# neuroailab/CounterfactualWorldModels

Measured on AMD Instinct MI355X. Metric: predicted frames/sec (2x224x224, ViT-B/8), higher is better.
Workload: dtype bf16; 1 GPU; ViT-base VMAE 8x8, batch=32 synthetic frame pairs (BASELINE configs[1]); predictor=base_8x8patch_2frames_1tube, per_gpu_batch=32, global_batch=32, n_vis=792, mode=parity, lanes=2 (the batch runs as two half batches on two HIP streams inside the library), arithmetic=split-bf16 (hi+lo) MFMA operands, 3 MFMAs/product, fp32 accumulate, parallelism=dp1 (independent frame pairs per rank, no collective), weights=random-init (deterministic synthetic generator)

## Files before the change

counterfactualworldmodels_amd/csrc/attention.hip:

```cpp
#include "attention_tail.h"

namespace cwm {

template <int PLANES>
__global__ __launch_bounds__(256, 2) void attention_kernel(const AttnParams p) {
    constexpr int TILE_BYTES = 64 * 64 * 2;
    constexpr int STAGE_BYTES = TILE_BYTES * 2 * PLANES;
    extern __shared__ __attribute__((aligned(16))) char smem[];

    const int tid = threadIdx.x;
    const int lane = tid & 63;
    const int wave = __builtin_amdgcn_readfirstlane(tid >> 6);
    const int qcol = lane & 31, hh = lane >> 5;
    const int N = p.n_tok;
    int qt, bh;
    attn_tile_of_block(p.n_q > 0 ? p.n_q : p.n_tok, 128, p.remap != 0, qt, bh);
    if (attention_is_split_tail(p, qt, gridDim.x, p.n_q > 0 ? p.n_q : p.n_tok)) {
        attention_tail_block<PLANES>(p, smem, bh, qt * 128, p.n_q > 0 ? p.n_q : p.n_tok);
        return;
    }
    const int b = bh / p.heads, h = bh - b * p.heads;
    const int q0 = qt * 128 + wave * 32;
    const int NQ = p.n_q > 0 ? p.n_q : p.n_tok;
    const bool active = q0 < NQ;
// ... 45 lines not shown
#pragma unroll
                for (int pl = 0; pl < PLANES; ++pl) kfr[kb][s][pl] = *reinterpret_cast<const bf16x8*>(base + pl * TILE_BYTES + k_off[kb][s]);
        __builtin_amdgcn_sched_barrier(0);
        f32x16 sacc[2];
#pragma unroll
        for (int kb = 0; kb < 2; ++kb) {
#pragma unroll
            for (int r = 0; r < 16; ++r) sacc[kb][r] = 0.f;
#pragma unroll
            for (int s = 0; s < 4; ++s) mfma_split<PLANES>(sacc[kb], kfr[kb][s][0], kfr[kb][s][PLANES - 1], qf[0][s], qf[PLANES - 1][s]);
        }
        __builtin_amdgcn_sched_barrier(0);
        bf16x4 vfr[4][2][PLANES][2];
#pragma unroll
        for (int ks = 0; ks < 4; ++ks)
#pragma unroll
            for (int db = 0; db < 2; ++db)
#pragma unroll
                for (int pl = 0; pl < PLANES; ++pl) {
                    const char* vb = base + (PLANES + pl) * TILE_BYTES + v_base[db] + ks * 2048;
                    vfr[ks][db][pl][0] = lds_read_tr16(vb);
                    vfr[ks][db][pl][1] = lds_read_tr16(vb + 1024);
                }
        __builtin_amdgcn_sched_barrier(0);

        if constexpr (LAST) {
            if (N & 63) {
#pragma unroll
                for (int kb = 0; kb < 2; ++kb) mask_rows_from(sacc[kb], kt * 64 + kb * 32, hh, N);
            }
        }
        float mx = sacc[0][0];
#pragma unroll
        for (int kb = 0; kb < 2; ++kb)
#pragma unroll
            for (int r = 0; r < 16; ++r) mx = fmaxf(mx, sacc[kb][r]);
        mx = max_lane_xor32(mx);
        const float m_new = fmaxf(m_run, mx);
        const bool grew = __any(m_new > m_run);
        const float alpha = grew ? __builtin_amdgcn_exp2f((m_run - m_new) * kLog2e) : 1.0f;
        m_run = m_new;
        const float mc = m_new * kLog2e;
        float rowsum = 0.f;
#pragma unroll
        for (int kb = 0; kb < 2; ++kb)
#pragma unroll
            for (int r = 0; r < 16; ++r) {
                const float pv = __builtin_amdgcn_exp2f(fmaf(sacc[kb][r], kLog2e, -mc));
                sacc[kb][r] = pv;
                rowsum += pv;
            }
        l_run = l_run * alpha + rowsum;
        if (grew) {
#pragma unroll
            for (int db = 0; db < 2; ++db)
#pragma unroll
                for (int r = 0; r < 16; ++r) oacc[db][r] *= alpha;
        }

#pragma unroll
        for (int ks = 0; ks < 4; ++ks) {
            const int kb = ks >> 1, s = ks & 1;
            bf16x8 ph, plo;
            p_fragments<PLANES>(sacc[kb], s, ph, plo);
#pragma unroll
            for (int db = 0; db < 2; ++db) mfma_split<PLANES>(oacc[db], join_halves(vfr[ks][db][0]), join_halves(vfr[ks][db][PLANES - 1]), ph, plo);
        }
        }

        if constexpr (!LAST) {
            store_tiles(cur ^ 1);
            __syncthreads();
        }
    };
    for (int kt = 0; kt + 1 < nkt; ++kt) tile_step(kt, std::false_type{});
    tile_step(nkt - 1, std::true_type{});

    const float l_tot = l_run + __shfl_xor(l_run, 32, 64);
    const float inv = 1.0f / l_tot;
    const int q = q0 + qcol;
    if (q < NQ) {
        const int64_t orow = (int64_t)b * NQ + q;
#pragma unroll
        for (int db = 0; db < 2; ++db) store_o_block<PLANES>(p.o, orow, p.ldo, h * 64 + db * 32, oacc[db], inv, hh);
    }
}

int launch_attention(const AttnParams& p_in, int planes, hipStream_t stream) {
    AttnParams p = p_in;
    const Tuning& tn = p.tune ? *p.tune : default_tuning();
    p.remap = tn.attn_remap;
    p.tail_split = tn.attn_tail;
    CWM_REQUIRE(planes == 1 || planes == 2, "attention: planes must be 1 or 2");
    CWM_REQUIRE(p.n_tok > 0 && p.batch > 0 && p.heads > 0, "attention: empty problem");
    CWM_REQUIRE(p.ldo % 4 == 0, "attention: ldo must be a multiple of 4");
    CWM_REQUIRE((int64_t)p.n_tok * 128 < (1ll << 31), "attention: %d tokens exceed the 32-bit tile offsets within one (batch, head)", p.n_tok);
    CWM_REQUIRE(p.q_off >= 0 && p.n_q >= 0 && p.q_off + p.n_q <= p.n_tok, "attention: query rows [%d, %d) outside the %d tokens", p.q_off, p.q_off + p.n_q, p.n_tok);
    const int nqb = ((p.n_q > 0 ? p.n_q : p.n_tok) + 127) / 128;
    const int kern = tn.attn_kernel ? tn.attn_kernel : (p.n_tok >= (planes == 2 ? 160 : 512) ? 3 : 1);
    if (kern == 3) return launch_attention_pipe(p, planes, stream);
    CWM_REQUIRE(kern == 1, "attention: unknown kernel %d (1: 4-wave, 3: software-pipelined)", kern);
    const dim3 grid(nqb, p.batch * p.heads);
    const size_t smem = (size_t)2 * (64 * 64 * 2) * 2 * planes;
    if (planes == 1) {
        hipLaunchKernelGGL(attention_kernel<1>, grid, dim3(256), smem, stream, p);
    } else {
        if (int rc = cwm_set_max_lds((const void*)attention_kernel<2>, (int)smem)) return rc;
        hipLaunchKernelGGL(attention_kernel<2>, grid, dim3(256), smem, stream, p);
    }
    CWM_HIP_CHECK(hipGetLastError());
    return 0;
}

}
```

counterfactualworldmodels_amd/csrc/attention_device.h:

```cpp
#pragma once
#include "common.h"
#include "kernels.h"
#include <type_traits>

namespace cwm {

__device__ __forceinline__ void attn_tile_of_item(int L, int nqb, int nbh, int nq, int rows, bool remap, int& qt, int& bh) {
    qt = L % nqb;
    bh = L / nqb;
    if (nbh % 8 != 0 || !remap) return;
    const int xcd = L & 7, idx = L >> 3, per = nbh >> 3;
    const int light = (nqb > 1 && (nq - (nqb - 1) * rows) * 2 <= rows) ? 1 : 0;
    const int heavy = nqb - light;
    if (idx < per * heavy) {
        bh = xcd * per + idx / heavy;
        qt = idx - (idx / heavy) * heavy;
    } else {
        bh = xcd * per + (idx - per * heavy);
        qt = nqb - 1;
    }
}
__device__ __forceinline__ void attn_tile_of_block(int nq, int rows, bool remap, int& qt, int& bh) {
    attn_tile_of_item(blockIdx.y * gridDim.x + blockIdx.x, gridDim.x, gridDim.y, nq, rows, remap, qt, bh);
}

__device__ __forceinline__ int lds_off128(int row, int chunk) { return row * 128 + ((chunk ^ ((row >> 1) & 7)) << 4); }
__device__ __forceinline__ int lds_off_v(int row, int chunk) { return row * 128 + ((chunk ^ (((row >> 1) & 1) << 2)) << 4); }

typedef __attribute__((ext_vector_type(4))) short s16x4;
__device__ __forceinline__ bf16x4 lds_read_tr16(const char* ptr) {
    typedef __attribute__((address_space(3))) s16x4 lds_s16x4;
    const s16x4 v = __builtin_amdgcn_ds_read_tr16_b64_v4i16((lds_s16x4*)ptr);
    return __builtin_bit_cast(bf16x4, v);
}
__device__ __forceinline__ bf16x8 join_halves(const bf16x4 (&h)[2]) { return __builtin_shufflevector(h[0], h[1], 0, 1, 2, 3, 4, 5, 6, 7); }

typedef __attribute__((ext_vector_type(2))) unsigned int u32x2;
template <int OFF>
__device__ __forceinline__ u32x2 lds_read_tr16_asm(unsigned addr) {
    u32x2 v;
    asm volatile("ds_read_b64_tr_b16 %0, %1 offset:%2" : "=v"(v) : "v"(addr), "n"(OFF) : "memory");
    return v;
}
template <int KS, int PLANES>
__device__ __forceinline__ void lds_read_v_step(u32x2 (&dst)[2][PLANES][2], unsigned va0, unsigned va1) {
    constexpr int T = 64 * 64 * 2;
    dst[0][0][0] = lds_read_tr16_asm<KS * 2048>(va0);
    dst[0][0][1] = lds_read_tr16_asm<KS * 2048 + 1024>(va0);
    if constexpr (PLANES == 2) {
        dst[0][PLANES - 1][0] = lds_read_tr16_asm<KS * 2048 + T>(va0);
        dst[0][PLANES - 1][1] = lds_read_tr16_asm<KS * 2048 + T + 1024>(va0);
    }
    dst[1][0][0] = lds_read_tr16_asm<KS * 2048>(va1);
    dst[1][0][1] = lds_read_tr16_asm<KS * 2048 + 1024>(va1);
    if constexpr (PLANES == 2) {
        dst[1][PLANES - 1][0] = lds_read_tr16_asm<KS * 2048 + T>(va1);
        dst[1][PLANES - 1][1] = lds_read_tr16_asm<KS * 2048 + T + 1024>(va1);
    }
}

template <int N, int PLANES>
__device__ __forceinline__ void lds_wait_v_step(u32x2 (&v)[2][PLANES][2]) {
    if constexpr (PLANES == 2)
        asm volatile("s_waitcnt lgkmcnt(%8)"
                     : "+v"(v[0][0][0]), "+v"(v[0][0][1]), "+v"(v[0][1][0]), "+v"(v[0][1][1]), "+v"(v[1][0][0]), "+v"(v[1][0][1]), "+v"(v[1][1][0]), "+v"(v[1][1][1])
                     : "n"(N)
                     : "memory");
    else
        asm volatile("s_waitcnt lgkmcnt(%4)" : "+v"(v[0][0][0]), "+v"(v[0][0][1]), "+v"(v[1][0][0]), "+v"(v[1][0][1]) : "n"(N) : "memory");
}

__device__ __forceinline__ float max_lane_xor32(float x) {
    const auto sw = __builtin_amdgcn_permlane32_swap(__float_as_uint(x), __float_as_uint(x), false, false);
    return fmaxf(__uint_as_float(sw[0]), __uint_as_float(sw[1]));
}

__device__ __forceinline__ float sum_lane_xor32(float x) {
    const auto sw = __builtin_amdgcn_permlane32_swap(__float_as_uint(x), __float_as_uint(x), false, false);
    return __uint_as_float(sw[0]) + __uint_as_float(sw[1]);
}


template <int PLANES>
__device__ __forceinline__ void mfma_split(f32x16& acc, const bf16x8& a_hi, const bf16x8& a_lo, const bf16x8& b_hi, const bf16x8& b_lo) {
    if constexpr (PLANES == 2) {
        acc = __builtin_amdgcn_mfma_f32_32x32x16_bf16(a_lo, b_hi, acc, 0, 0, 0);
        acc = __builtin_amdgcn_mfma_f32_32x32x16_bf16(a_hi, b_lo, acc, 0, 0, 0);
    }
    acc = __builtin_amdgcn_mfma_f32_32x32x16_bf16(a_hi, b_hi, acc, 0, 0, 0);
}

template <int PLANES>
__device__ __forceinline__ void p_fragments(const f32x16& s, int ks, bf16x8& ph, bf16x8& plo) {
#pragma unroll
    for (int j = 0; j < 8; ++j) split_bf16_at<PLANES>(s[8 * ks + j], ph, plo, j);
}

__device__ __forceinline__ int acc_row(int r, int hh) { return (r & 3) + 8 * (r >> 2) + 4 * hh; }
__device__ __forceinline__ void mask_rows_from(f32x16& s, int row0, int hh, int limit) {
#pragma unroll
    for (int r = 0; r < 16; ++r)
        if (row0 + acc_row(r, hh) >= limit) s[r] = -INFINITY;
}

template <int PLANES>
__device__ __forceinline__ void store_o_block(bf16* o, int64_t row, int ld, int col0, const f32x16& acc, float mul, int hh) {
#pragma unroll
    for (int g = 0; g < 4; ++g) {
        bf16x4 hi4, lo4;
#pragma unroll
        for (int e = 0; e < 4; ++e) split_bf16_at<PLANES>(acc[4 * g + e] * mul, hi4, lo4, e);
        store_operand_split<PLANES>(o, row, ld, col0 + 8 * g + 4 * hh, hi4, lo4);
    }
}

template <int PLANES>
__device__ __forceinline__ void load_q_fragments(bf16x8 (&qf)[PLANES][4], const bf16* Qb, int64_t qk_plane, int qrow, int hh) {
#pragma unroll
    for (int pl = 0; pl < PLANES; ++pl)
#pragma unroll
        for (int s = 0; s < 4; ++s) qf[pl][s] = *reinterpret_cast<const bf16x8*>(Qb + (size_t)pl * qk_plane + (size_t)qrow * 64 + s * 16 + hh * 8);
}

__device__ __forceinline__ int v_tr_offset(int lane, int db) {
    const int g = lane >> 4, q = (lane >> 2) & 3, pc = lane & 3;
    return lds_off_v(4 * (g >> 1) + q, db * 4 + (g & 1) * 2 + (pc >> 1)) + (pc & 1) * 8;
}

template <int PLANES, int NT>
struct KvStage {
    static constexpr int TILE_BYTES = 64 * 64 * 2;
    int row[2], chunk[2], koff[2], voff[2];
    u32x4 rk[NT][PLANES][2], rv[NT][PLANES][2];
    __device__ __forceinline__ void init(int tid) {
#pragma unroll
        for (int i = 0; i < 2; ++i) {
            const int idx = tid + i * 256;
            row[i] = idx >> 3;
            chunk[i] = idx & 7;
            koff[i] = lds_off128(row[i], chunk[i]);
            voff[i] = lds_off_v(row[i], chunk[i]);
        }
    }
    __device__ __forceinline__ void load(int t, const bf16* Kb, const bf16* Vb, int64_t qk_plane, int kt, int N) {
#pragma unroll
        for (int i = 0; i < 2; ++i) {
            const size_t off = (size_t)min(kt * 64 + row[i], N - 1) * 64 + chunk[i] * 8;
#pragma unroll
            for (int pl = 0; pl < PLANES; ++pl) {
                rk[t][pl][i] = *reinterpret_cast<const u32x4*>(Kb + (size_t)pl * qk_plane + off);
                rv[t][pl][i] = *reinterpret_cast<const u32x4*>(Vb + (size_t)pl * qk_plane + off);
            }
        }
    }
    __device__ __forceinline__ void store(int t, char* stage) const {
#pragma unroll
        for (int i = 0; i < 2; ++i)
#pragma unroll
            for (int pl = 0; pl < PLANES; ++pl) {
                *reinterpret_cast<u32x4*>(stage + pl * TILE_BYTES + koff[i]) = rk[t][pl][i];
                *reinterpret_cast<u32x4*>(stage + (PLANES + pl) * TILE_BYTES + voff[i]) = rv[t][pl][i];
            }
    }
};

}
```

counterfactualworldmodels_amd/csrc/attention_pipe.hip:

```cpp
#include "attention_tail.h"
#include <algorithm>
#include <cstdio>
#include <map>
#include <mutex>
#include <utility>

namespace cwm {

#ifdef CWM_ATTN_PROF
__device__ unsigned long long g_pipe_prof[8];
__device__ unsigned long long g_pipe_blocks[8192 * 8];
#define PROF_T(i) do { if (prof) { const unsigned long long t_ = __builtin_amdgcn_s_memtime(); pacc[i] += t_ - tlast; tlast = t_; } } while (0)
#else
#define PROF_T(i) do {} while (0)
#endif

namespace {

constexpr float kLog2e = 1.4426950408889634f;
constexpr int kKsplitMaxWgs = 512;

template <int PLANES>
struct PipeWave {
    bf16x8 qf[PLANES][4];
    f32x16 oacc[2];
    float m_run, l_run;
    int k_off[2][4];
    int hh;
};

template <int PLANES>
__device__ __forceinline__ void qk_plain(const PipeWave<PLANES>& w, const char* kbase, f32x16 (&s)[2]) {
    constexpr int TILE_BYTES = 64 * 64 * 2;
#pragma unroll
    for (int kb = 0; kb < 2; ++kb) {
#pragma unroll
        for (int r = 0; r < 16; ++r) s[kb][r] = 0.f;
#pragma unroll
        for (int sx = 0; sx < 4; ++sx) {
            bf16x8 kf[PLANES];
#pragma unroll
            for (int pl = 0; pl < PLANES; ++pl) kf[pl] = *reinterpret_cast<const bf16x8*>(kbase + pl * TILE_BYTES + w.k_off[kb][sx]);
            mfma_split<PLANES>(s[kb], kf[0], kf[PLANES - 1], w.qf[0][sx], w.qf[PLANES - 1][sx]);
        }
    }
}

template <int PLANES>
__device__ __forceinline__ void split_pair(const f32x16 (&sc)[2], int ks, int j, bf16x8& ph, bf16x8& plo) {
#pragma unroll
    for (int e = 2 * j; e < 2 * j + 2; ++e) {
        split_bf16_at<PLANES>(sc[ks >> 1][8 * (ks & 1) + e], ph, plo, e);
    }
}

template <int PLANES, int KS>
__device__ __forceinline__ void pv_step(PipeWave<PLANES>& w, const f32x16 (&sc)[2], const u32x2 (&vr)[2][PLANES][2], const bf16x8& ph, const bf16x8& plo,
                                        bf16x8& ph_next, bf16x8& plo_next) {
    constexpr int NM = PLANES == 2 ? 3 : 1;
    constexpr int NSLOT = 2 * NM;
    bf16x8 vf[2], vl[2];
#pragma unroll
    for (int db = 0; db < 2; ++db) {
        vf[db] = __builtin_shufflevector(__builtin_bit_cast(bf16x4, vr[db][0][0]), __builtin_bit_cast(bf16x4, vr[db][0][1]), 0, 1, 2, 3, 4, 5, 6, 7);
        if constexpr (PLANES == 2)
            vl[db] = __builtin_shufflevector(__builtin_bit_cast(bf16x4, vr[db][PLANES - 1][0]), __builtin_bit_cast(bf16x4, vr[db][PLANES - 1][1]), 0, 1, 2, 3, 4, 5, 6, 7);
    }
#pragma unroll
    for (int m = 0; m < NM; ++m)
#pragma unroll
        for (int db = 0; db < 2; ++db) {
            const int slot = m * 2 + db;
            if constexpr (PLANES == 2) {
                if (m == 0) w.oacc[db] = __builtin_amdgcn_mfma_f32_32x32x16_bf16(vl[db], ph, w.oacc[db], 0, 0, 0);
                if (m == 1) w.oacc[db] = __builtin_amdgcn_mfma_f32_32x32x16_bf16(vf[db], plo, w.oacc[db], 0, 0, 0);
                if (m == 2) w.oacc[db] = __builtin_amdgcn_mfma_f32_32x32x16_bf16(vf[db], ph, w.oacc[db], 0, 0, 0);
            } else {
                w.oacc[db] = __builtin_amdgcn_mfma_f32_32x32x16_bf16(vf[db], ph, w.oacc[db], 0, 0, 0);
            }
            if constexpr (KS < 3) {
#pragma unroll
                for (int j = 0; j < 4; ++j)
                    if (j * NSLOT / 4 == slot) split_pair<PLANES>(sc, KS + 1, j, ph_next, plo_next);
            }
            __builtin_amdgcn_sched_barrier(0);
        }
}

enum : int { TILE_STEADY = 0, TILE_PENULT = 1, TILE_LAST = 2 };
template <int PLANES, int KIND, int NDMA, typename Dma>
__device__ __forceinline__ void pipe_tile(PipeWave<PLANES>& w, f32x16 (&sc)[2], f32x16 (&sn)[2], const char* kbase, unsigned va0, unsigned va1, int kt, int N, bool half_next,
                                          bool half_this, Dma&& dma
#ifdef CWM_ATTN_PROF
    , bool prof, unsigned long long (&pacc)[8], unsigned long long& tlast
#endif
    ) {
    constexpr bool HAS_NEXT = KIND != TILE_LAST;
    constexpr bool LASTK = KIND == TILE_LAST;
    constexpr int TILE_BYTES = 64 * 64 * 2;
    constexpr int NM = PLANES == 2 ? 3 : 1;
    constexpr int NS = 8 * NM;
    constexpr int NMAX = NS / 4;
    constexpr int NE = NS - NMAX - 1;
    constexpr int NRD = 4 * PLANES;

    if constexpr (LASTK) {
        if (N & 63) {
#pragma unroll
            for (int kb = 0; kb < 2; ++kb) mask_rows_from(sc[kb], kt * 64 + kb * 32, w.hh, N);
        }
    }

    bf16x8 kfr[8][PLANES];
    auto read_k = [&](int g) {
        const int kb = g & 1, sx = g >> 1;
#pragma unroll
        for (int pl = 0; pl < PLANES; ++pl) kfr[g][pl] = *reinterpret_cast<const bf16x8*>(kbase + pl * TILE_BYTES + w.k_off[kb][sx]);
    };
    if constexpr (HAS_NEXT) {
        read_k(0);
        read_k(1);
#pragma unroll
        for (int kb = 0; kb < 2; ++kb)
#pragma unroll
            for (int r = 0; r < 16; ++r) sn[kb][r] = 0.f;
    }
    float mx = sc[0][0];
    float m_new = 0.f, alpha = 1.f, mc = 0.f, rowsum = 0.f;
    bool grew = false;
    u32x2 vr0[2][PLANES][2], vr1[2][PLANES][2];
    bf16x8 ph0, pl0, ph1, pl1;
#pragma unroll
    for (int g = 0; g < 8; ++g) {
        const int kb = g & 1, sx = g >> 1;
        if constexpr (HAS_NEXT) {
            if (g + 2 < 8) read_k(g + 2);
        }
#pragma unroll
        for (int m = 0; m < NM; ++m) {
            const int slot = g * NM + m;
            if (slot < NDMA) dma(slot);
            if (HAS_NEXT && !(kb == 1 && half_next && slot < NS - 1)) {
                if constexpr (PLANES == 2) {
                    if (m == 0) sn[kb] = __builtin_amdgcn_mfma_f32_32x32x16_bf16(kfr[g][PLANES - 1], w.qf[0][sx], sn[kb], 0, 0, 0);
                    if (m == 1) sn[kb] = __builtin_amdgcn_mfma_f32_32x32x16_bf16(kfr[g][0], w.qf[PLANES - 1][sx], sn[kb], 0, 0, 0);
                    if (m == 2) sn[kb] = __builtin_amdgcn_mfma_f32_32x32x16_bf16(kfr[g][0], w.qf[0][sx], sn[kb], 0, 0, 0);
                } else {
                    sn[kb] = __builtin_amdgcn_mfma_f32_32x32x16_bf16(kfr[g][0], w.qf[0][sx], sn[kb], 0, 0, 0);
                }
            }
            if (slot < NMAX) {
#pragma unroll
                for (int v = 32 * slot / NMAX; v < 32 * (slot + 1) / NMAX; ++v) mx = fmaxf(mx, sc[v >> 4][v & 15]);
            } else if (slot == NMAX) {
                mx = max_lane_xor32(mx);
                m_new = fmaxf(w.m_run, mx);
                grew = __any(m_new > w.m_run);
                alpha = grew ? __builtin_amdgcn_exp2f((w.m_run - m_new) * kLog2e) : 1.0f;
                w.m_run = m_new;
                mc = m_new * kLog2e;
                if (KIND == TILE_LAST || grew) {
#pragma unroll
                    for (int db = 0; db < 2; ++db)
#pragma unroll
                        for (int r = 0; r < 16; ++r) w.oacc[db][r] *= alpha;
                }
            } else {
                const int j = slot - NMAX - 1;
                if (j > 0) {
#pragma unroll
                    for (int v = 32 * (j - 1) / NE; v < 32 * j / NE; ++v) rowsum += sc[v >> 4][v & 15];
                }
#pragma unroll
                for (int v = 32 * j / NE; v < 32 * (j + 1) / NE; ++v) sc[v >> 4][v & 15] = __builtin_amdgcn_exp2f(fmaf(sc[v >> 4][v & 15], kLog2e, -mc));
                asm volatile("" : "+v"(rowsum));
            }
            if (slot >= NS - 4) split_pair<PLANES>(sc, 0, slot - (NS - 4), ph0, pl0);
            if (slot == NS - 2) lds_read_v_step<0, PLANES>(vr0, va0, va1);
            if (slot == NS - 1) lds_read_v_step<1, PLANES>(vr1, va0, va1);
            __builtin_amdgcn_sched_barrier(0);
        }
    }

    PROF_T(1);
#pragma unroll
    for (int v = 32 * (NE - 1) / NE; v < 32; ++v) rowsum += sc[v >> 4][v & 15];
    w.l_run = w.l_run * alpha + rowsum;
    __builtin_amdgcn_sched_barrier(0);
    lds_wait_v_step<NRD, PLANES>(vr0);
    pv_step<PLANES, 0>(w, sc, vr0, ph0, pl0, ph1, pl1);
    if constexpr (LASTK) {
        lds_wait_v_step<0, PLANES>(vr1);
        pv_step<PLANES, 1>(w, sc, vr1, ph1, pl1, ph0, pl0);
        if (!half_this) {
            lds_read_v_step<2, PLANES>(vr0, va0, va1);
            lds_read_v_step<3, PLANES>(vr1, va0, va1);
            lds_wait_v_step<NRD, PLANES>(vr0);
            pv_step<PLANES, 2>(w, sc, vr0, ph0, pl0, ph1, pl1);
            lds_wait_v_step<0, PLANES>(vr1);
            pv_step<PLANES, 3>(w, sc, vr1, ph1, pl1, ph0, pl0);
        }
    } else {
        lds_read_v_step<2, PLANES>(vr0, va0, va1);
        lds_wait_v_step<NRD, PLANES>(vr1);
        pv_step<PLANES, 1>(w, sc, vr1, ph1, pl1, ph0, pl0);
        lds_read_v_step<3, PLANES>(vr1, va0, va1);
        lds_wait_v_step<NRD, PLANES>(vr0);
        pv_step<PLANES, 2>(w, sc, vr0, ph0, pl0, ph1, pl1);
        lds_wait_v_step<0, PLANES>(vr1);
        pv_step<PLANES, 3>(w, sc, vr1, ph1, pl1, ph0, pl0);
    }
    PROF_T(2);
}

}

template <int PLANES, int NW>
__global__ __launch_bounds__(64 * NW, NW == 4 ? 2 : 1) void attention_pipe_kernel(const AttnParams p) {
    constexpr int TILE_BYTES = 64 * 64 * 2;
    constexpr int SLOT_BYTES = TILE_BYTES * PLANES;
    constexpr int V_BASE = 2 * SLOT_BYTES;
    constexpr int NP = 8 * PLANES / NW;
    extern __shared__ __attribute__((aligned(16))) char smem[];
    typedef __attribute__((address_space(3))) void lds_void;
    typedef const __attribute__((address_space(1))) void gbl_void;

    const int tid = threadIdx.x;
    const int lane = tid & 63;
    const int wave = __builtin_amdgcn_readfirstlane(tid >> 6);
    const int qcol = lane & 31, hh = lane >> 5;
    const int N = p.n_tok;
    const int NQ = p.n_q > 0 ? p.n_q : N;
    const int nkt_all = (N + 63) / 64;
    int item = blockIdx.x, kt0 = 0, nkt = nkt_all, part = -1;
    if (p.ks_parts > 0 && item >= p.ks_main) {
        const int sidx = item - p.ks_main;
        item = p.ks_main + sidx / p.ks_parts;
        part = sidx - (sidx / p.ks_parts) * p.ks_parts;
        kt0 = nkt_all * part / p.ks_parts;
        nkt = nkt_all * (part + 1) / p.ks_parts;
    }
    int qt, bh;
    attn_tile_of_item(item, p.ks_nqb, p.batch * p.heads, NQ, 32 * NW, p.remap != 0, qt, bh);
    if constexpr (NW == 4) {
        if (attention_is_split_tail(p, qt, p.ks_nqb, NQ)) {
            attention_tail_block<PLANES>(p, smem, bh, qt * 128, NQ);
            return;
        }
    }
    const int b = bh / p.heads, h = bh - b * p.heads;
    const int q0 = qt * (32 * NW) + wave * 32;
    const bool active = q0 < NQ;

    const bf16* Qb = p.q + (size_t)bh * N * 64;
    const bf16* Kb = p.k + (size_t)bh * N * 64;
    const bf16* Vb = p.v + (size_t)bh * N * 64;

    PipeWave<PLANES> w;
    w.hh = hh;
    load_q_fragments<PLANES>(w.qf, Qb, p.qk_plane, p.q_off + min(q0 + qcol, NQ - 1), hh);

    int st_lds[NP], st_koff[NP], st_voff[NP];
    const char *st_kp[NP], *st_vp[NP];
#pragma unroll
    for (int jj = 0; jj < NP; ++jj) {
        const int pi = wave * NP + jj, plane = pi >> 3, pc = pi & 7;
        const int r = pc * 8 + (lane >> 3);
        st_lds[jj] = plane * TILE_BYTES + pc * 1024;
        st_koff[jj] = r * 128 + ((lane & 7) ^ ((r >> 1) & 7)) * 16;
        st_voff[jj] = r * 128 + ((lane & 7) ^ (((r >> 1) & 1) << 2)) * 16;
        st_kp[jj] = reinterpret_cast<const char*>(Kb + (size_t)plane * p.qk_plane);
        st_vp[jj] = reinterpret_cast<const char*>(Vb + (size_t)plane * p.qk_plane);
    }
    auto tile_off = [&](int kt, int toff, auto clamp_c) -> unsigned {
        if constexpr (decltype(clamp_c)::value) return (unsigned)(min(kt * 64 + (toff >> 7), N - 1) * 128 + (toff & 127));
        else return (unsigned)(kt * 8192 + toff);
    };
    auto stage_k1 = [&](int kt, int slot, int jj, auto clamp_c) {
        __builtin_amdgcn_global_load_lds((gbl_void*)(st_kp[jj] + tile_off(kt, st_koff[jj], clamp_c)), (lds_void*)(smem + slot * SLOT_BYTES + st_lds[jj]), 16, 0, 0);
    };
    auto stage_v1 = [&](int kt, int slot, int jj, auto clamp_c) {
        __builtin_amdgcn_global_load_lds((gbl_void*)(st_vp[jj] + tile_off(kt, st_voff[jj], clamp_c)), (lds_void*)(smem + V_BASE + slot * SLOT_BYTES + st_lds[jj]), 16, 0,
                                         0);
    };
    auto stage_k = [&](int kt, int slot) {
#pragma unroll
        for (int jj = 0; jj < NP; ++jj) stage_k1(kt, slot, jj, std::true_type{});
    };
    auto stage_v = [&](int kt, int slot) {
#pragma unroll
        for (int jj = 0; jj < NP; ++jj) stage_v1(kt, slot, jj, std::true_type{});
    };

#pragma unroll
    for (int kb = 0; kb < 2; ++kb)
#pragma unroll
        for (int s = 0; s < 4; ++s) w.k_off[kb][s] = lds_off128(kb * 32 + qcol, 2 * s + hh);
    unsigned v_addr[2];
#pragma unroll
    for (int db = 0; db < 2; ++db) v_addr[db] = (unsigned)(size_t)(lds_void*)(smem + V_BASE + v_tr_offset(lane, db));

#pragma unroll
    for (int db = 0; db < 2; ++db)
#pragma unroll
        for (int r = 0; r < 16; ++r) w.oacc[db][r] = 0.f;
    w.m_run = -1e30f;
    w.l_run = 0.f;

#define CWM_TILE_END()                                     \
    do {                                                   \
        asm volatile("s_waitcnt vmcnt(0)" ::: "memory");   \
        __builtin_amdgcn_sched_barrier(0);                 \
        __builtin_amdgcn_s_barrier();                      \
        __builtin_amdgcn_sched_barrier(0);                 \
    } while (0)
#define CWM_TILE(KIND, SC, SN, KT, CLAMP)                                                                                              \
    do {                                                                                                                               \
        const int kt_ = (KT);                                                                                                          \
        const int ks_ = kt_ & 1;                                                                                                       \
        auto dma = [&](int i) {                                                                                                        \
            if (i < NP) {                                                                                                              \
                if ((KIND) == TILE_STEADY) stage_k1(kt_ + 2, ks_, i, CLAMP);                                                           \
            } else if ((KIND) != TILE_LAST) {                                                                                          \
                stage_v1(kt_ + 1, ks_ ^ 1, i - NP, CLAMP);                                                                             \
            }                                                                                                                          \
        };                                                                                                                             \
        PROF_T(0);                                                                                                                     \
        if (active) {                                                                                                                  \
            pipe_tile<PLANES, KIND, 2 * NP>(w, SC, SN, smem + (ks_ ^ 1) * SLOT_BYTES, v_addr[0] + ks_ * SLOT_BYTES, v_addr[1] + ks_ * SLOT_BYTES, kt_, N,  \
                                            (KIND) == TILE_PENULT && half_last, half_last, dma PROF_ARGS);                             \
        } else {                                                                                                                       \
            if ((KIND) == TILE_STEADY) stage_k(kt_ + 2, ks_);                                                                          \
            if ((KIND) != TILE_LAST) stage_v(kt_ + 1, ks_ ^ 1);                                                                        \
        }                                                                                                                              \
        if ((KIND) != TILE_LAST) CWM_TILE_END();                                                                                       \
        PROF_T(3);                                                                                                                     \
    } while (0)

#ifdef CWM_ATTN_PROF
#define PROF_ARGS , prof, pacc, tlast
    const bool prof = wave == 0;
    unsigned long long pacc[8] = {0, 0, 0, 0, 0, 0, 0, 0};
    unsigned long long tlast = __builtin_amdgcn_s_memtime();
    const unsigned long long t_begin = tlast, r_begin = __builtin_amdgcn_s_memrealtime();
#else
#define PROF_ARGS
#endif
    const bool half_last = nkt == nkt_all && ((N - 1) & 63) < 32;

    auto store_out = [&]() {
        const float l_tot = w.l_run + __shfl_xor(w.l_run, 32, 64);
        const int q = q0 + qcol;
        if (part >= 0) {
            if (q < NQ) {
                float* rec = p.ks_scratch + (((size_t)(item - p.ks_main) * p.ks_parts + part) * 128 + (wave * 32 + qcol)) * 68;
#pragma unroll
                for (int db = 0; db < 2; ++db)
#pragma unroll
                    for (int g = 0; g < 4; ++g)
                        *reinterpret_cast<f32x4*>(rec + db * 32 + 8 * g + 4 * hh) =
                            f32x4{w.oacc[db][4 * g], w.oacc[db][4 * g + 1], w.oacc[db][4 * g + 2], w.oacc[db][4 * g + 3]};
                if (hh == 0) {
                    rec[64] = w.m_run;
                    rec[65] = l_tot;
                }
            }
            return;
        }
        const float inv = 1.0f / l_tot;
        if (q < NQ) {
            const int64_t orow = (int64_t)b * NQ + q;
#pragma unroll
            for (int db = 0; db < 2; ++db) store_o_block<PLANES>(p.o, orow, p.ldo, h * 64 + db * 32, w.oacc[db], inv, hh);
        }
    };

    f32x16 sa[2], sb[2];
    stage_k(kt0, kt0 & 1);
    stage_v(kt0, kt0 & 1);
    if (kt0 + 1 < nkt) stage_k(kt0 + 1, (kt0 + 1) & 1);
    CWM_TILE_END();
    if (active) qk_plain<PLANES>(w, smem + (kt0 & 1) * SLOT_BYTES, sa);
    __builtin_amdgcn_sched_barrier(0);
    __builtin_amdgcn_s_barrier();
    __builtin_amdgcn_sched_barrier(0);

    int kt = kt0;
    const int n_mine = nkt - kt0;
    if (n_mine >= 3) {
        for (; kt + 4 < nkt; kt += 2) {
            CWM_TILE(TILE_STEADY, sa, sb, kt, std::false_type{});
            CWM_TILE(TILE_STEADY, sb, sa, kt + 1, std::false_type{});
        }
        for (;;) {
            CWM_TILE(TILE_STEADY, sa, sb, kt, std::true_type{});
            ++kt;
            if (kt + 2 == nkt) break;
#pragma unroll
            for (int kb = 0; kb < 2; ++kb) sa[kb] = sb[kb];
        }
    } else if (n_mine == 2) {
#pragma unroll
        for (int kb = 0; kb < 2; ++kb) sb[kb] = sa[kb];
    }
    if (n_mine >= 2) {
        CWM_TILE(TILE_PENULT, sb, sa, kt, std::true_type{});
        ++kt;
    }
    CWM_TILE(TILE_LAST, sa, sb, kt, std::true_type{});
    store_out();
#undef CWM_TILE
#undef CWM_TILE_END
#ifdef CWM_ATTN_PROF
    pacc[4] = __builtin_amdgcn_s_memtime() - t_begin;
    pacc[5] = __builtin_amdgcn_s_memrealtime() - r_begin;
    {
        const int bid = blockIdx.x;
        if (wave == 0 && lane == 0 && bid < 8192) {
            g_pipe_blocks[bid * 8 + 0] = r_begin;
            g_pipe_blocks[bid * 8 + 1] = r_begin + pacc[5];
            g_pipe_blocks[bid * 8 + 2] = pacc[4];
            g_pipe_blocks[bid * 8 + 3] = __builtin_amdgcn_s_getreg((4 << 0) | (0 << 6) | (31 << 11));
            for (int i = 0; i < 4; ++i) g_pipe_blocks[bid * 8 + 4 + i] = pacc[i];
        }
    }
    if (prof && lane == 0 && blockIdx.x == 0 && blockIdx.y == 0)
        for (int i = 0; i < 8; ++i) g_pipe_prof[i] = pacc[i];
#endif
}

#ifdef CWM_ATTN_PROF
int attention_pipe_prof(int i) {
    if (i >= 1000) {
        static unsigned long long h[8192 * 8];
        if (hipMemcpyFromSymbol(h, HIP_SYMBOL(g_pipe_blocks), sizeof(h)) != hipSuccess) return -1;
        FILE* f = fopen("/tmp/attn_blocks.bin", "wb");
        if (!f) return -1;
        fwrite(h, 1, sizeof(h), f);
        fclose(f);
        return 0;
    }
    unsigned long long h[8];
    if (hipMemcpyFromSymbol(h, HIP_SYMBOL(g_pipe_prof), sizeof(h)) != hipSuccess) return -1;
    return (int)h[i & 7];
}
#else
int attention_pipe_prof(int) { return -1; }
#endif

template <int PLANES>
__global__ __launch_bounds__(256) void attention_combine_kernel(const AttnParams p) {
    const int wave = threadIdx.x >> 6, d = threadIdx.x & 63;
    const int N = p.n_tok, NQ = p.n_q > 0 ? p.n_q : N;
    const int sitem = blockIdx.x / 32, qrow = (blockIdx.x % 32) * 4 + wave;
    int qt, bh;
    attn_tile_of_item(p.ks_main + sitem, p.ks_nqb, p.batch * p.heads, NQ, 128, p.remap != 0, qt, bh);
    const int q = qt * 128 + qrow;
    if (q >= NQ) return;
    const float* rec = p.ks_scratch + (((size_t)sitem * p.ks_parts) * 128 + qrow) * 68;
    float m = -INFINITY;
    for (int j = 0; j < p.ks_parts; ++j) m = fmaxf(m, rec[(size_t)j * 128 * 68 + 64]);
    float o = 0.f, l = 0.f;
    for (int j = 0; j < p.ks_parts; ++j) {
        const float* r = rec + (size_t)j * 128 * 68;
        const float wgt = __builtin_amdgcn_exp2f((r[64] - m) * kLog2e);
        o = fmaf(r[d], wgt, o);
        l = fmaf(r[65], wgt, l);
    }
    const float v = o / l;
    const int b = bh / p.heads, h = bh - b * p.heads;
    store_operand<PLANES>(p.o, (int64_t)b * NQ + q, p.ldo, h * 64 + d, v);
}

static int ksplit_scratch(hipStream_t stream, float** out) {
    static std::mutex mu;
    static std::map<std::pair<int, hipStream_t>, float*> table;
    int dev = 0;
    CWM_HIP_CHECK(hipGetDevice(&dev));
    std::lock_guard<std::mutex> lock(mu);
    auto it = table.find(std::make_pair(dev, stream));
    if (it == table.end()) {
        float* buf = nullptr;
        CWM_HIP_CHECK(hipMalloc((void**)&buf, (size_t)kKsplitMaxWgs * 128 * 68 * sizeof(float)));
        it = table.emplace(std::make_pair(dev, stream), buf).first;
    }
    *out = it->second;
    return 0;
}

template <int PLANES, int NW>
static int launch_pipe(const AttnParams& p_in, hipStream_t stream) {
    AttnParams p = p_in;
// ... 42 lines not shown
```

counterfactualworldmodels_amd/csrc/attention_tail.h:

```cpp
#pragma once
#include "attention_device.h"

namespace cwm {

template <int PLANES>
__device__ __forceinline__ void attention_tail_block(const AttnParams& p, char* smem, int bh, int q0, int NQ) {
    constexpr int TILE_BYTES = 64 * 64 * 2;
    constexpr int STAGE_BYTES = TILE_BYTES * 2 * PLANES;
    constexpr float kLog2eT = 1.4426950408889634f;
    const int tid = threadIdx.x, lane = tid & 63;
    const int wave = __builtin_amdgcn_readfirstlane(tid >> 6);
    const int qcol = lane & 31, hh = lane >> 5;
    const int N = p.n_tok;
    const int b = bh / p.heads, h = bh - b * p.heads;
    const int kb = wave & 1, slot = wave >> 1;

    const bf16* Qb = p.q + (size_t)bh * N * 64;
    const bf16* Kb = p.k + (size_t)bh * N * 64;
    const bf16* Vb = p.v + (size_t)bh * N * 64;

    bf16x8 qf[PLANES][4];
    load_q_fragments<PLANES>(qf, Qb, p.qk_plane, p.q_off + min(q0 + qcol, NQ - 1), hh);
    const int nkt = (N + 63) / 64, npass = (nkt + 1) / 2;
    KvStage<PLANES, 2> st;
// ... 37 lines not shown
            }
            bf16x4 vfr[2][2][PLANES][2];
#pragma unroll
            for (int ks = 0; ks < 2; ++ks)
#pragma unroll
                for (int db = 0; db < 2; ++db)
#pragma unroll
                    for (int pl = 0; pl < PLANES; ++pl) {
                        const char* vb = base + (PLANES + pl) * TILE_BYTES + v_base[db] + (kb * 2 + ks) * 2048;
                        vfr[ks][db][pl][0] = lds_read_tr16(vb);
                        vfr[ks][db][pl][1] = lds_read_tr16(vb + 1024);
                    }
            if (kt == nkt - 1 && (N & 63)) mask_rows_from(sacc, kt * 64 + kb * 32, hh, N);
            float mx = sacc[0];
#pragma unroll
            for (int r = 1; r < 16; ++r) mx = fmaxf(mx, sacc[r]);
            mx = max_lane_xor32(mx);
            const float m_new = fmaxf(m_run, mx);
            const float alpha = __builtin_amdgcn_exp2f((m_run - m_new) * kLog2eT);
            m_run = m_new;
            const float mc = m_new * kLog2eT;
            float rowsum = 0.f;
#pragma unroll
            for (int r = 0; r < 16; ++r) {
                const float pv = __builtin_amdgcn_exp2f(fmaf(sacc[r], kLog2eT, -mc));
                sacc[r] = pv;
                rowsum += pv;
            }
            l_run = l_run * alpha + rowsum;
#pragma unroll
            for (int db = 0; db < 2; ++db)
#pragma unroll
                for (int r = 0; r < 16; ++r) oacc[db][r] *= alpha;
#pragma unroll
            for (int ks = 0; ks < 2; ++ks) {
                bf16x8 ph, plo;
                p_fragments<PLANES>(sacc, ks, ph, plo);
#pragma unroll
                for (int db = 0; db < 2; ++db) mfma_split<PLANES>(oacc[db], join_halves(vfr[ks][db][0]), join_halves(vfr[ks][db][PLANES - 1]), ph, plo);
            }
        }
        if (pass + 1 < npass) load_pair(pass + 1);
        __syncthreads();
        if (pass + 1 < npass) {
            store_pair();
            __syncthreads();
        }
    }

    float* mbuf = reinterpret_cast<float*>(smem);
    auto put = [&](int w2) {
        float* d = mbuf + (size_t)w2 * 34 * 64 + lane;
#pragma unroll
        for (int db = 0; db < 2; ++db)
#pragma unroll
            for (int r = 0; r < 16; ++r) d[(db * 16 + r) * 64] = oacc[db][r];
        d[32 * 64] = m_run;
        d[33 * 64] = l_run;
    };
    auto take = [&](int w2) {
        const float* s = mbuf + (size_t)w2 * 34 * 64 + lane;
        const float m_o = s[32 * 64], l_o = s[33 * 64];
        const float m_new = fmaxf(m_run, m_o);
        const float fa = __builtin_amdgcn_exp2f((m_run - m_new) * kLog2eT), fb = __builtin_amdgcn_exp2f((m_o - m_new) * kLog2eT);
#pragma unroll
        for (int db = 0; db < 2; ++db)
#pragma unroll
            for (int r = 0; r < 16; ++r) oacc[db][r] = fmaf(oacc[db][r], fa, s[(db * 16 + r) * 64] * fb);
        l_run = fmaf(l_run, fa, l_o * fb);
        m_run = m_new;
    };
    if (wave >= 2) put(wave - 2);
    __syncthreads();
    if (wave < 2) take(wave);
    __syncthreads();
    if (wave == 1) put(0);
    __syncthreads();
    if (wave != 0) return;
    take(0);

    const float l_tot = l_run + __shfl_xor(l_run, 32, 64);
    const float inv = 1.0f / l_tot;
    const int q = q0 + qcol;
    if (q < NQ) {
        const int64_t orow = (int64_t)b * NQ + q;
#pragma unroll
        for (int db = 0; db < 2; ++db) store_o_block<PLANES>(p.o, orow, p.ldo, h * 64 + db * 32, oacc[db], inv, hh);
    }
}

__device__ __forceinline__ bool attention_is_split_tail(const AttnParams& p, int qt, int nqb, int NQ) {
    const int rows = NQ - qt * 128;
    return p.tail_split && nqb > 1 && qt == nqb - 1 && rows <= 32 && p.n_tok > 128;
}

}
```

Baseline: 1970 frames/s.

## Use constant LDS offsets in pipelined attention and widen output stores

The pipelined attention kernel now computes K/V LDS addresses as a base plus compile-time immediate offsets, with the unrolled steady-state loop using fixed slot indices. This removes per-tile address arithmetic and registers. The P split uses packed bf16x2 conversion plus inline v_sub/v_max3, and the row-max reduction uses max3. The output store pairs groups across lane halves with permlane32_swap so each lane writes 8 bf16 at a time instead of 4. The added inline asm and offset constraints make the code more fragile to compiler scheduling.

```diff
diff --git a/counterfactualworldmodels_amd/csrc/attention.hip b/counterfactualworldmodels_amd/csrc/attention.hip
--- a/counterfactualworldmodels_amd/csrc/attention.hip
+++ b/counterfactualworldmodels_amd/csrc/attention.hip
@@ -151,7 +151,14 @@
     if (q < NQ) {
         const int64_t orow = (int64_t)b * NQ + q;
 #pragma unroll
-        for (int db = 0; db < 2; ++db) store_o_block<PLANES>(p.o, orow, p.ldo, h * 64 + db * 32, oacc[db], inv, hh);
+        for (int db = 0; db < 2; ++db)
+#pragma unroll
+            for (int g = 0; g < 4; ++g) {
+                bf16x4 hi4, lo4;
+#pragma unroll
+                for (int e = 0; e < 4; ++e) split_bf16_at<PLANES>(oacc[db][4 * g + e] * inv, hi4, lo4, e);
+                store_operand_split<PLANES>(p.o, orow, p.ldo, h * 64 + db * 32 + 8 * g + 4 * hh, hi4, lo4);
+            }
     }
 }
 
diff --git a/counterfactualworldmodels_amd/csrc/attention_device.h b/counterfactualworldmodels_amd/csrc/attention_device.h
--- a/counterfactualworldmodels_amd/csrc/attention_device.h
+++ b/counterfactualworldmodels_amd/csrc/attention_device.h
@@ -42,20 +42,22 @@
     asm volatile("ds_read_b64_tr_b16 %0, %1 offset:%2" : "=v"(v) : "v"(addr), "n"(OFF) : "memory");
     return v;
 }
-template <int KS, int PLANES>
+template <int KS, int PLANES, int BASE = 0>
 __device__ __forceinline__ void lds_read_v_step(u32x2 (&dst)[2][PLANES][2], unsigned va0, unsigned va1) {
     constexpr int T = 64 * 64 * 2;
-    dst[0][0][0] = lds_read_tr16_asm<KS * 2048>(va0);
-    dst[0][0][1] = lds_read_tr16_asm<KS * 2048 + 1024>(va0);
+    constexpr int O = BASE + KS * 2048;
+    static_assert(O + T + 1024 < 65536, "immediate offset of an LDS read is 16 bits");
+    dst[0][0][0] = lds_read_tr16_asm<O>(va0);
+    dst[0][0][1] = lds_read_tr16_asm<O + 1024>(va0);
     if constexpr (PLANES == 2) {
-        dst[0][PLANES - 1][0] = lds_read_tr16_asm<KS * 2048 + T>(va0);
-        dst[0][PLANES - 1][1] = lds_read_tr16_asm<KS * 2048 + T + 1024>(va0);
+        dst[0][PLANES - 1][0] = lds_read_tr16_asm<O + T>(va0);
+        dst[0][PLANES - 1][1] = lds_read_tr16_asm<O + T + 1024>(va0);
     }
-    dst[1][0][0] = lds_read_tr16_asm<KS * 2048>(va1);
-    dst[1][0][1] = lds_read_tr16_asm<KS * 2048 + 1024>(va1);
+    dst[1][0][0] = lds_read_tr16_asm<O>(va1);
+    dst[1][0][1] = lds_read_tr16_asm<O + 1024>(va1);
     if constexpr (PLANES == 2) {
-        dst[1][PLANES - 1][0] = lds_read_tr16_asm<KS * 2048 + T>(va1);
-        dst[1][PLANES - 1][1] = lds_read_tr16_asm<KS * 2048 + T + 1024>(va1);
+        dst[1][PLANES - 1][0] = lds_read_tr16_asm<O + T>(va1);
+        dst[1][PLANES - 1][1] = lds_read_tr16_asm<O + T + 1024>(va1);
     }
 }
 
@@ -78,6 +80,17 @@
 __device__ __forceinline__ float sum_lane_xor32(float x) {
     const auto sw = __builtin_amdgcn_permlane32_swap(__float_as_uint(x), __float_as_uint(x), false, false);
     return __uint_as_float(sw[0]) + __uint_as_float(sw[1]);
+}
+
+__device__ __forceinline__ float sub_f32_single(float a, float b) {
+    float d;
+    asm("v_sub_f32 %0, %1, %2" : "=v"(d) : "v"(a), "v"(b));
+    return d;
+}
+__device__ __forceinline__ float max3_f32_single(float a, float b, float c) {
+    float d;
+    asm("v_max3_f32 %0, %1, %2, %3" : "=v"(d) : "v"(a), "v"(b), "v"(c));
+    return d;
 }
 
 
@@ -103,14 +116,26 @@
         if (row0 + acc_row(r, hh) >= limit) s[r] = -INFINITY;
 }
 
+__device__ __forceinline__ bf16x8 pair_groups_xor32(const bf16x4& a, const bf16x4& b) {
+    const u32x2 ua = __builtin_bit_cast(u32x2, a), ub = __builtin_bit_cast(u32x2, b);
+    const auto x = __builtin_amdgcn_permlane32_swap(ua[0], ub[0], false, false);
+    const auto y = __builtin_amdgcn_permlane32_swap(ua[1], ub[1], false, false);
+    return __builtin_bit_cast(bf16x8, u32x4{x[0], y[0], x[1], y[1]});
+}
+
 template <int PLANES>
-__device__ __forceinline__ void store_o_block(bf16* o, int64_t row, int ld, int col0, const f32x16& acc, float mul, int hh) {
+__device__ __forceinline__ void store_o_block(bf16* o, int64_t row, int ld, int col0, const f32x16& acc, float mul, int hh, bool ok) {
 #pragma unroll
-    for (int g = 0; g < 4; ++g) {
-        bf16x4 hi4, lo4;
+    for (int g = 0; g < 4; g += 2) {
+        bf16x4 hi4[2], lo4[2];
 #pragma unroll
-        for (int e = 0; e < 4; ++e) split_bf16_at<PLANES>(acc[4 * g + e] * mul, hi4, lo4, e);
-        store_operand_split<PLANES>(o, row, ld, col0 + 8 * g + 4 * hh, hi4, lo4);
+        for (int t = 0; t < 2; ++t)
+#pragma unroll
+            for (int e = 0; e < 4; ++e) split_bf16_at<PLANES>(acc[4 * (g + t) + e] * mul, hi4[t], lo4[t], e);
+        const bf16x8 hi8 = pair_groups_xor32(hi4[0], hi4[1]);
+        bf16x8 lo8;
+        if constexpr (PLANES == 2) lo8 = pair_groups_xor32(lo4[0], lo4[1]);
+        if (ok) store_operand_split<PLANES>(o, row, ld, col0 + 8 * g + 8 * hh, hi8, lo8);
     }
 }
 
diff --git a/counterfactualworldmodels_amd/csrc/attention_pipe.hip b/counterfactualworldmodels_amd/csrc/attention_pipe.hip
--- a/counterfactualworldmodels_amd/csrc/attention_pipe.hip
+++ b/counterfactualworldmodels_amd/csrc/attention_pipe.hip
@@ -25,12 +25,19 @@
     bf16x8 qf[PLANES][4];
     f32x16 oacc[2];
     float m_run, l_run;
-    int k_off[2][4];
+    unsigned k_addr[4];
     int hh;
 };
 
+constexpr int K_BLOCK1 = 32 * 128;
+template <int OFF>
+__device__ __forceinline__ bf16x8 lds_read_k(unsigned addr) {
+    typedef const __attribute__((address_space(3))) bf16x8 lds_bf16x8;
+    return *reinterpret_cast<lds_bf16x8*>((size_t)(addr + OFF));
+}
+
 template <int PLANES>
-__device__ __forceinline__ void qk_plain(const PipeWave<PLANES>& w, const char* kbase, f32x16 (&s)[2]) {
+__device__ __forceinline__ void qk_plain(const PipeWave<PLANES>& w, f32x16 (&s)[2]) {
     constexpr int TILE_BYTES = 64 * 64 * 2;
 #pragma unroll
     for (int kb = 0; kb < 2; ++kb) {
@@ -40,25 +47,33 @@
         for (int sx = 0; sx < 4; ++sx) {
             bf16x8 kf[PLANES];
 #pragma unroll
-            for (int pl = 0; pl < PLANES; ++pl) kf[pl] = *reinterpret_cast<const bf16x8*>(kbase + pl * TILE_BYTES + w.k_off[kb][sx]);
+            for (int pl = 0; pl < PLANES; ++pl) kf[pl] = kb ? (pl ? lds_read_k<K_BLOCK1 + TILE_BYTES>(w.k_addr[sx]) : lds_read_k<K_BLOCK1>(w.k_addr[sx]))
+                                                                   : (pl ? lds_read_k<TILE_BYTES>(w.k_addr[sx]) : lds_read_k<0>(w.k_addr[sx]));
             mfma_split<PLANES>(s[kb], kf[0], kf[PLANES - 1], w.qf[0][sx], w.qf[PLANES - 1][sx]);
         }
     }
 }
 
+typedef __attribute__((ext_vector_type(2))) float f32x2;
 template <int PLANES>
-__device__ __forceinline__ void split_pair(const f32x16 (&sc)[2], int ks, int j, bf16x8& ph, bf16x8& plo) {
-#pragma unroll
-    for (int e = 2 * j; e < 2 * j + 2; ++e) {
-        split_bf16_at<PLANES>(sc[ks >> 1][8 * (ks & 1) + e], ph, plo, e);
+__device__ __forceinline__ void split_pair(const f32x16 (&sc)[2], int ks, int j, u32x4& ph, u32x4& plo) {
+    const float a = sc[ks >> 1][8 * (ks & 1) + 2 * j], b = sc[ks >> 1][8 * (ks & 1) + 2 * j + 1];
+    const unsigned h = __builtin_bit_cast(unsigned, __builtin_convertvector(f32x2{a, b}, bf16x2));
+    ph[j] = h;
+    if constexpr (PLANES == 2) {
+        const float la = sub_f32_single(a, __uint_as_float(h << 16)), lb = sub_f32_single(b, __uint_as_float(h & 0xffff0000u));
+        plo[j] = __builtin_bit_cast(unsigned, __builtin_convertvector(f32x2{la, lb}, bf16x2));
     }
 }
 
 template <int PLANES, int KS>
-__device__ __forceinline__ void pv_step(PipeWave<PLANES>& w, const f32x16 (&sc)[2], const u32x2 (&vr)[2][PLANES][2], const bf16x8& ph, const bf16x8& plo,
-                                        bf16x8& ph_next, bf16x8& plo_next) {
+__device__ __forceinline__ void pv_step(PipeWave<PLANES>& w, const f32x16 (&sc)[2], const u32x2 (&vr)[2][PLANES][2], const u32x4& ph_, const u32x4& plo_,
+                                        u32x4& ph_next, u32x4& plo_next) {
     constexpr int NM = PLANES == 2 ? 3 : 1;
     constexpr int NSLOT = 2 * NM;
+    const bf16x8 ph = __builtin_bit_cast(bf16x8, ph_);
+    bf16x8 plo;
+    if constexpr (PLANES == 2) plo = __builtin_bit_cast(bf16x8, plo_);
     bf16x8 vf[2], vl[2];
 #pragma unroll
     for (int db = 0; db < 2; ++db) {
@@ -88,8 +103,8 @@
 }
 
 enum : int { TILE_STEADY = 0, TILE_PENULT = 1, TILE_LAST = 2 };
-template <int PLANES, int KIND, int NDMA, typename Dma>
-__device__ __forceinline__ void pipe_tile(PipeWave<PLANES>& w, f32x16 (&sc)[2], f32x16 (&sn)[2], const char* kbase, unsigned va0, unsigned va1, int kt, int N, bool half_next,
+template <int PLANES, int KIND, int NDMA, int KS, typename Dma>
+__device__ __forceinline__ void pipe_tile(PipeWave<PLANES>& w, f32x16 (&sc)[2], f32x16 (&sn)[2], unsigned kofs, unsigned va0, unsigned va1, int kt, int N, bool half_next,
                                           bool half_this, Dma&& dma
 #ifdef CWM_ATTN_PROF
     , bool prof, unsigned long long (&pacc)[8], unsigned long long& tlast
@@ -103,6 +118,8 @@
     constexpr int NMAX = NS / 4;
     constexpr int NE = NS - NMAX - 1;
     constexpr int NRD = 4 * PLANES;
+    constexpr int SLOT_BYTES = TILE_BYTES * PLANES;
+    constexpr int KOFF = KS < 0 ? 0 : (KS ^ 1) * SLOT_BYTES, VOFF = KS < 0 ? 0 : KS * SLOT_BYTES;
 
     if constexpr (LASTK) {
         if (N & 63) {
@@ -115,7 +132,10 @@
     auto read_k = [&](int g) {
         const int kb = g & 1, sx = g >> 1;
 #pragma unroll
-        for (int pl = 0; pl < PLANES; ++pl) kfr[g][pl] = *reinterpret_cast<const bf16x8*>(kbase + pl * TILE_BYTES + w.k_off[kb][sx]);
+        for (int pl = 0; pl < PLANES; ++pl) {
+            const unsigned a = KS < 0 ? w.k_addr[sx] + kofs : w.k_addr[sx];
+            kfr[g][pl] = kb ? (pl ? lds_read_k<KOFF + K_BLOCK1 + TILE_BYTES>(a) : lds_read_k<KOFF + K_BLOCK1>(a)) : (pl ? lds_read_k<KOFF + TILE_BYTES>(a) : lds_read_k<KOFF>(a));
+        }
     };
     if constexpr (HAS_NEXT) {
         read_k(0);
@@ -129,7 +149,7 @@
     float m_new = 0.f, alpha = 1.f, mc = 0.f, rowsum = 0.f;
     bool grew = false;
     u32x2 vr0[2][PLANES][2], vr1[2][PLANES][2];
-    bf16x8 ph0, pl0, ph1, pl1;
+    u32x4 ph0, pl0, ph1, pl1;
 #pragma unroll
     for (int g = 0; g < 8; ++g) {
         const int kb = g & 1, sx = g >> 1;
@@ -150,8 +170,9 @@
                 }
             }
             if (slot < NMAX) {
-#pragma unroll
-                for (int v = 32 * slot / NMAX; v < 32 * (slot + 1) / NMAX; ++v) mx = fmaxf(mx, sc[v >> 4][v & 15]);
+                const int V0 = 32 * slot / NMAX > 1 ? 32 * slot / NMAX : 1, V1 = 32 * (slot + 1) / NMAX;
+#pragma unroll
+                for (int v = V0; v < V1; v += 2) mx = max3_f32_single(mx, sc[v >> 4][v & 15], sc[(v + 1 < V1 ? v + 1 : v) >> 4][(v + 1 < V1 ? v + 1 : v) & 15]);
             } else if (slot == NMAX) {
                 mx = max_lane_xor32(mx);
                 m_new = fmaxf(w.m_run, mx);
@@ -176,8 +197,8 @@
                 asm volatile("" : "+v"(rowsum));
             }
             if (slot >= NS - 4) split_pair<PLANES>(sc, 0, slot - (NS - 4), ph0, pl0);
-            if (slot == NS - 2) lds_read_v_step<0, PLANES>(vr0, va0, va1);
-            if (slot == NS - 1) lds_read_v_step<1, PLANES>(vr1, va0, va1);
+            if (slot == NS - 2) lds_read_v_step<0, PLANES, VOFF>(vr0, va0, va1);
+            if (slot == NS - 1) lds_read_v_step<1, PLANES, VOFF>(vr1, va0, va1);
             __builtin_amdgcn_sched_barrier(0);
         }
     }
@@ -193,18 +214,18 @@
         lds_wait_v_step<0, PLANES>(vr1);
         pv_step<PLANES, 1>(w, sc, vr1, ph1, pl1, ph0, pl0);
         if (!half_this) {
-            lds_read_v_step<2, PLANES>(vr0, va0, va1);
-            lds_read_v_step<3, PLANES>(vr1, va0, va1);
+            lds_read_v_step<2, PLANES, VOFF>(vr0, va0, va1);
+            lds_read_v_step<3, PLANES, VOFF>(vr1, va0, va1);
             lds_wait_v_step<NRD, PLANES>(vr0);
             pv_step<PLANES, 2>(w, sc, vr0, ph0, pl0, ph1, pl1);
             lds_wait_v_step<0, PLANES>(vr1);
             pv_step<PLANES, 3>(w, sc, vr1, ph1, pl1, ph0, pl0);
         }
     } else {
-        lds_read_v_step<2, PLANES>(vr0, va0, va1);
+        lds_read_v_step<2, PLANES, VOFF>(vr0, va0, va1);
         lds_wait_v_step<NRD, PLANES>(vr1);
         pv_step<PLANES, 1>(w, sc, vr1, ph1, pl1, ph0, pl0);
-        lds_read_v_step<3, PLANES>(vr1, va0, va1);
+        lds_read_v_step<3, PLANES, VOFF>(vr1, va0, va1);
         lds_wait_v_step<NRD, PLANES>(vr0);
         pv_step<PLANES, 2>(w, sc, vr0, ph0, pl0, ph1, pl1);
         lds_wait_v_step<0, PLANES>(vr1);
@@ -272,16 +293,18 @@
         st_kp[jj] = reinterpret_cast<const char*>(Kb + (size_t)plane * p.qk_plane);
         st_vp[jj] = reinterpret_cast<const char*>(Vb + (size_t)plane * p.qk_plane);
     }
-    auto tile_off = [&](int kt, int toff, auto clamp_c) -> unsigned {
-        if constexpr (decltype(clamp_c)::value) return (unsigned)(min(kt * 64 + (toff >> 7), N - 1) * 128 + (toff & 127));
-        else return (unsigned)(kt * 8192 + toff);
+    auto tile_ptr = [&](const char* base, int kt, int& toff, auto clamp_c) -> const char* {
+        if constexpr (decltype(clamp_c)::value) return base + (unsigned)(min(kt * 64 + (toff >> 7), N - 1) * 128 + (toff & 127));
+        else {
+            asm volatile("" : "+v"(toff));
+            return (base + (size_t)kt * 8192) + (unsigned)toff;
+        }
     };
     auto stage_k1 = [&](int kt, int slot, int jj, auto clamp_c) {
-        __builtin_amdgcn_global_load_lds((gbl_void*)(st_kp[jj] + tile_off(kt, st_koff[jj], clamp_c)), (lds_void*)(smem + slot * SLOT_BYTES + st_lds[jj]), 16, 0, 0);
+        __builtin_amdgcn_global_load_lds((gbl_void*)tile_ptr(st_kp[jj], kt, st_koff[jj], clamp_c), (lds_void*)(smem + slot * SLOT_BYTES + st_lds[jj]), 16, 0, 0);
     };
     auto stage_v1 = [&](int kt, int slot, int jj, auto clamp_c) {
-        __builtin_amdgcn_global_load_lds((gbl_void*)(st_vp[jj] + tile_off(kt, st_voff[jj], clamp_c)), (lds_void*)(smem + V_BASE + slot * SLOT_BYTES + st_lds[jj]), 16, 0,
-                                         0);
+        __builtin_amdgcn_global_load_lds((gbl_void*)tile_ptr(st_vp[jj], kt, st_voff[jj], clamp_c), (lds_void*)(smem + V_BASE + slot * SLOT_BYTES + st_lds[jj]), 16, 0, 0);
     };
     auto stage_k = [&](int kt, int slot) {
 #pragma unroll
@@ -293,9 +316,10 @@
     };
 
 #pragma unroll
-    for (int kb = 0; kb < 2; ++kb)
-#pragma unroll
-        for (int s = 0; s < 4; ++s) w.k_off[kb][s] = lds_off128(kb * 32 + qcol, 2 * s + hh);
+    for (int s = 0; s < 4; ++s) {
+        w.k_addr[s] = (unsigned)(size_t)(lds_void*)(smem + lds_off128(qcol, 2 * s + hh));
+        asm volatile("" : "+v"(w.k_addr[s]));
+    }
     unsigned v_addr[2];
 #pragma unroll
     for (int db = 0; db < 2; ++db) v_addr[db] = (unsigned)(size_t)(lds_void*)(smem + V_BASE + v_tr_offset(lane, db));
@@ -314,10 +338,12 @@
         __builtin_amdgcn_s_barrier();                      \
         __builtin_amdgcn_sched_barrier(0);                 \
     } while (0)
-#define CWM_TILE(KIND, SC, SN, KT, CLAMP)                                                                                              \
+#define CWM_TILE(KIND, SC, SN, KT, KS, CLAMP)                                                                                          \
     do {                                                                                                                               \
         const int kt_ = (KT);                                                                                                          \
-        const int ks_ = kt_ & 1;                                                                                                       \
+        constexpr int ksc_ = (KS);                                                                                                     \
+        const int ks_ = ksc_ >= 0 ? ksc_ : ((kt_ - kt0) & 1);                                                                          \
+        const int ro_ = ksc_ >= 0 ? 0 : SLOT_BYTES;               \
         auto dma = [&](int i) {                                                                                                        \
             if (i < NP) {                                                                                                              \
                 if ((KIND) == TILE_STEADY) stage_k1(kt_ + 2, ks_, i, CLAMP);                                                           \
@@ -327,8 +353,8 @@
         };                                                                                                                             \
         PROF_T(0);                                                                                                                     \
         if (active) {                                                                                                                  \
-            pipe_tile<PLANES, KIND, 2 * NP>(w, SC, SN, smem + (ks_ ^ 1) * SLOT_BYTES, v_addr[0] + ks_ * SLOT_BYTES, v_addr[1] + ks_ * SLOT_BYTES, kt_, N,  \
-                                            (KIND) == TILE_PENULT && half_last, half_last, dma PROF_ARGS);                             \
+            pipe_tile<PLANES, KIND, 2 * NP, ksc_>(w, SC, SN, (ks_ ^ 1) * ro_, v_addr[0] + ks_ * ro_, v_addr[1] + ks_ * ro_, kt_, N,             \
+                                                  (KIND) == TILE_PENULT && half_last, half_last, dma PROF_ARGS);                       \
         } else {                                                                                                                       \
             if ((KIND) == TILE_STEADY) stage_k(kt_ + 2, ks_);                                                                          \
             if ((KIND) != TILE_LAST) stage_v(kt_ + 1, ks_ ^ 1);                                                                        \
@@ -349,7 +375,7 @@
     const bool half_last = nkt == nkt_all && ((N - 1) & 63) < 32;
 
     auto store_out = [&]() {
-        const float l_tot = w.l_run + __shfl_xor(w.l_run, 32, 64);
+        const float l_tot = sum_lane_xor32(w.l_run);
         const int q = q0 + qcol;
         if (part >= 0) {
             if (q < NQ) {
@@ -368,19 +394,17 @@
             return;
         }
         const float inv = 1.0f / l_tot;
-        if (q < NQ) {
-            const int64_t orow = (int64_t)b * NQ + q;
-#pragma unroll
-            for (int db = 0; db < 2; ++db) store_o_block<PLANES>(p.o, orow, p.ldo, h * 64 + db * 32, w.oacc[db], inv, hh);
-        }
+        const int64_t orow = (int64_t)b * NQ + q;
+#pragma unroll
+        for (int db = 0; db < 2; ++db) store_o_block<PLANES>(p.o, orow, p.ldo, h * 64 + db * 32, w.oacc[db], inv, hh, q < NQ);
     };
 
     f32x16 sa[2], sb[2];
-    stage_k(kt0, kt0 & 1);
-    stage_v(kt0, kt0 & 1);
-    if (kt0 + 1 < nkt) stage_k(kt0 + 1, (kt0 + 1) & 1);
+    stage_k(kt0, 0);
+    stage_v(kt0, 0);
+    if (kt0 + 1 < nkt) stage_k(kt0 + 1, 1);
     CWM_TILE_END();
-    if (active) qk_plain<PLANES>(w, smem + (kt0 & 1) * SLOT_BYTES, sa);
+    if (active) qk_plain<PLANES>(w, sa);
     __builtin_amdgcn_sched_barrier(0);
     __builtin_amdgcn_s_barrier();
     __builtin_amdgcn_sched_barrier(0);
@@ -389,11 +413,11 @@
     const int n_mine = nkt - kt0;
     if (n_mine >= 3) {
         for (; kt + 4 < nkt; kt += 2) {
-            CWM_TILE(TILE_STEADY, sa, sb, kt, std::false_type{});
-            CWM_TILE(TILE_STEADY, sb, sa, kt + 1, std::false_type{});
+            CWM_TILE(TILE_STEADY, sa, sb, kt, 0, std::false_type{});
+            CWM_TILE(TILE_STEADY, sb, sa, kt + 1, 1, std::false_type{});
         }
         for (;;) {
-            CWM_TILE(TILE_STEADY, sa, sb, kt, std::true_type{});
+            CWM_TILE(TILE_STEADY, sa, sb, kt, -1, std::true_type{});
             ++kt;
             if (kt + 2 == nkt) break;
 #pragma unroll
@@ -404,10 +428,10 @@
         for (int kb = 0; kb < 2; ++kb) sb[kb] = sa[kb];
     }
     if (n_mine >= 2) {
-        CWM_TILE(TILE_PENULT, sb, sa, kt, std::true_type{});
+        CWM_TILE(TILE_PENULT, sb, sa, kt, -1, std::true_type{});
         ++kt;
     }
-    CWM_TILE(TILE_LAST, sa, sb, kt, std::true_type{});
+    CWM_TILE(TILE_LAST, sa, sb, kt, -1, std::true_type{});
     store_out();
 #undef CWM_TILE
 #undef CWM_TILE_END
diff --git a/counterfactualworldmodels_amd/csrc/attention_tail.h b/counterfactualworldmodels_amd/csrc/attention_tail.h
--- a/counterfactualworldmodels_amd/csrc/attention_tail.h
+++ b/counterfactualworldmodels_amd/csrc/attention_tail.h
@@ -143,11 +143,9 @@
     const float l_tot = l_run + __shfl_xor(l_run, 32, 64);
     const float inv = 1.0f / l_tot;
     const int q = q0 + qcol;
-    if (q < NQ) {
-        const int64_t orow = (int64_t)b * NQ + q;
+    const int64_t orow = (int64_t)b * NQ + q;
 #pragma unroll
-        for (int db = 0; db < 2; ++db) store_o_block<PLANES>(p.o, orow, p.ldo, h * 64 + db * 32, oacc[db], inv, hh);
-    }
+    for (int db = 0; db < 2; ++db) store_o_block<PLANES>(p.o, orow, p.ldo, h * 64 + db * 32, oacc[db], inv, hh, q < NQ);
 }
 
 __device__ __forceinline__ bool attention_is_split_tail(const AttnParams& p, int qt, int nqb, int NQ) {
```

After: 1963 frames/s, median of 2. No clear change (-0.3%).
